# TIGER-AI-Lab/AnyV2V

Hardware: AMD Instinct MI355X
Metric: frames/sec for 16fx512x512 DDIM-inversion+PnP-edit; spatial-attn MFMA % of peak (higher is better)
Workload: dtype f16; 1 GPU; BASELINE config 3 per GPU: 1 clip x 16f x 512x512, 50-step DDIM inversion (UNet B=1) + 50-step PnP edit (UNet B=3, cfg 9.0, conv+spatial+temporal injection on every step); a bench step = 1 inversion step + 1 edit step = 1/50 clip; I2VGen-XL 3D-UNet 1.42B params, random init; frames=16, hip_graphs=True, finite=True

## Files before the change

### anyv2v_amd/csrc/gemm_plan.cpp

```cpp
#include "gemm_plan.h"

const char* av_gemm_family_name(GemmFamily f) {
    static const char* const names[] = {"naive", "ws", "ws_ln", "mfma128", "big", "pp", "sw", "sw_streamk", "swh"};
    static_assert(sizeof(names) / sizeof(names[0]) == GEMM_FAMILY_COUNT, "one name per family");
    return names[f];
}

namespace {
bool aligned16(const void* p) { return (((uintptr_t)p) & 15) == 0; }
int ceil_div(int a, int b) { return (a + b - 1) / b; }

#define PLAN_FAIL(code, ...) do { anyv2v_set_error(__VA_ARGS__); p.status = code; return p; } while (0)
#define PLAN_CHECK(cond, ...) if (!(cond)) PLAN_FAIL(ANYV2V_EINVAL, __VA_ARGS__)

int ws_slab_cols(const AnyV2VGemmDesc& d) {
    if (d.C0 == 320) return 160;
    if (d.C0 == 512) return d.act == ACT_GEGLU ? 128 : (d.N == 512 ? 64 : 0);
    return 0;
}
bool ws_eligible(const AnyV2VGemmDesc& d) {
    const int ns = ws_slab_cols(d);
    if (d.ln_c1 != nullptr && (d.R != nullptr || (d.C0 == 512 && d.act != ACT_GEGLU))) return false;
    return d.mode == MODE_LINEAR && ns > 0 && d.C1 == 0 && d.N % ns == 0 && d.N / ns <= 32 &&
           (d.act == ACT_NONE || (d.act == ACT_GEGLU && d.R == nullptr)) && d.rowvec == nullptr && d.M > 0;
}

bool sw_eligible(const AnyV2VGemmDesc& d, int nk) {
    const bool geglu = d.act == ACT_GEGLU;
    return d.N % 320 == 0 && (geglu ? d.mode == MODE_LINEAR && d.R == nullptr && d.rowvec == nullptr : d.act == ACT_NONE) &&
           !(d.R != nullptr && d.rowvec != nullptr) && nk >= 2 && d.ldc % 8 == 0 && (d.R == nullptr || d.ldr % 8 == 0) &&
           (d.rowvec == nullptr || d.ldrv % 8 == 0);
}
size_t sw_sk_workspace(int blocks) { return (size_t)2 * blocks * AV_GEMM_BM * AV_GEMM_BN * sizeof(float); }
int sw_sk_blocks(int tiles, int nk, bool force) {
    const long long U = (long long)tiles * nk;
    if (U < 256 * 4 || U > (1ll << 22)) return force && U >= 8 ? (int)(U / 4 < 256 ? U / 4 : 256) : 0;
    if (force) return 256;
    const int rounds = (tiles + 255) / 256;
    const double eff = (double)tiles / (rounds * 256.0);
    return eff < 0.9 ? 256 : 0;
}

bool swh_eligible(const AnyV2VGemmDesc& d) {
    return d.mode == MODE_CONV2D && d.stride == 1 && d.up == 0 && d.asym == 0 && d.Hi == d.Ho && d.Wi == d.Wo &&
           (d.Wi == 16 || d.Wi == 32 || d.Wi == 64) && d.N % 320 == 0 && d.act == ACT_NONE && d.C0 % 64 == 0 && d.C1 % 64 == 0 &&
           !(d.R != nullptr && d.rowvec != nullptr) && d.ldc % 8 == 0 && (d.R == nullptr || d.ldr % 8 == 0) &&
           (d.rowvec == nullptr || d.ldrv % 8 == 0);
}

bool gn_shape_ok(const AnyV2VGemmDesc& d) {
    if (d.gn_groups <= 0 || d.gn_rows_per_group <= 0 || d.N % 160 != 0 || d.N % d.gn_groups != 0) return false;
    const int cg = d.N / d.gn_groups;
    return 40 % cg == 0 && d.M % 16 == 0 && d.gn_rows_per_group % 16 == 0 && d.M % d.gn_rows_per_group == 0 &&
           (d.act == ACT_NONE || d.act == ACT_SILU || d.act == ACT_GELU);
}

void persistent_grid(GemmPlan& p, const AnyV2VGemmDesc& d) {
    p.tilesN = d.N / AV_GEMM_BN;
    p.tiles = ceil_div(d.M, AV_GEMM_BM) * p.tilesN;
    p.grid = p.tiles < 256 ? p.tiles : 256;
}
void raster(GemmPlan& p, const AnyV2VGemmDesc& d) {
    const int code = (d.flags >> ANYV2V_GEMM_RASTER_SHIFT) & 7;
    static const int gm_of[8] = {0, 0, 4, 8, 16, 32, 2, 0};
    int gm = gm_of[code];
    if (code == 0 && p.tilesN >= 8 && p.tiles >= 512) gm = 8;
    if (gm > 0 && p.grid == 256 && p.tilesN % (32 / gm) == 0) {
        p.rast_gm = gm;
        p.rast_gn = 32 / gm;
        p.rast_sm = ceil_div(ceil_div(d.M, AV_GEMM_BM), gm);
        p.rast_sn = p.tilesN / p.rast_gn;
        p.rast_nfast = (d.flags & ANYV2V_GEMM_RASTER_NFAST) != 0;
    }
}

}

GemmPlan av_gemm_plan(const AnyV2VGemmDesc& d, int hinted_rows) {
    GemmPlan p = {};
    p.nf = 4;
    p.splits = p.tilesN = 1;
    auto take = [&p](GemmFamily family, const char* what) { p.family = family; p.gn_decline = what; return p; };
    PLAN_CHECK(d.A0 && d.W, "gemm: null A0/W/C");
    PLAN_CHECK(d.M > 0 && d.N > 0 && d.C0 > 0 && d.C1 >= 0, "gemm: bad M/N/C0/C1 (%d %d %d %d)", d.M, d.N, d.C0, d.C1);
    PLAN_CHECK(d.mode >= 0 && d.mode <= 2, "gemm: bad mode %d", d.mode);
    PLAN_CHECK(d.act >= 0 && d.act <= 4, "gemm: bad act %d", d.act);
    PLAN_CHECK(d.act != ACT_F32OUT || (d.rowvec == nullptr && d.R == nullptr && d.N % 4 == 0 && d.ldc % 4 == 0),
               "gemm: fp32 output supports bias only and needs N, ldc multiples of 4");
    PLAN_CHECK(d.asym == 0 || d.asym == 1, "gemm: asym must be 0 or 1");
    PLAN_CHECK(d.C1 == 0 || d.A1 != nullptr, "gemm: C1 > 0 but A1 is null");
    PLAN_CHECK(d.rowvec == nullptr || d.rowvec_div > 0, "gemm: rowvec needs rowvec_div > 0");
    if (d.mode == MODE_CONV2D) {
        PLAN_CHECK(d.Hi > 0 && d.Wi > 0 && d.Ho > 0 && d.Wo > 0 && (d.stride == 1 || d.stride == 2), "gemm: bad conv geometry");
        PLAN_CHECK(d.M % (d.Ho * d.Wo) == 0, "gemm: M not a multiple of Ho*Wo");
        PLAN_CHECK(d.up == 0 || d.up == 1, "gemm: up must be 0 or 1");
    }
    if (d.mode == MODE_TEMPORAL) { PLAN_CHECK(d.F > 0 && d.HW > 0 && d.M % (d.F * d.HW) == 0, "gemm: bad temporal geometry"); }
    const bool geglu = d.act == ACT_GEGLU;
    if (geglu) {
        PLAN_CHECK(d.N % 32 == 0, "gemm: GEGLU needs N %% 32 == 0");
        PLAN_CHECK(d.rowvec == nullptr, "gemm: GEGLU with rowvec unsupported");
    }
    p.taps = d.mode == MODE_LINEAR ? 1 : (d.mode == MODE_CONV2D ? 9 : 3);
    p.nk = p.taps * (d.C0 / 64 + d.C1 / 64);
    p.vec_epi = (((uintptr_t)d.bias & 7) == 0) && (((uintptr_t)d.rowvec & 7) == 0) && (d.ldrv % 4 == 0) && (d.N % 4 == 0);
    const int flags = d.flags, nk = p.nk;
    const bool glds = (flags & ANYV2V_GEMM_LDS_DMA) != 0;
    const bool fast = !(flags & ANYV2V_GEMM_NAIVE) && d.C0 % 64 == 0 && d.C1 % 64 == 0 && d.lda0 % 8 == 0 &&
                      (d.C1 == 0 || d.lda1 % 8 == 0) && d.ldc % 8 == 0 && aligned16(d.A0) && (d.C1 == 0 || aligned16(d.A1)) &&
                      aligned16(d.W) && aligned16(d.C) && (d.R == nullptr || (d.ldr % 8 == 0 && aligned16(d.R))) &&
                      (!geglu || d.N % 128 == 0) && p.vec_epi;

    const bool ws_ok = fast && glds && ws_eligible(d);
    const bool ws_take = ws_ok && !(flags & (ANYV2V_GEMM_NO_WS | ANYV2V_GEMM_NO_BIG)) && (hinted_rows >= 32768 || (flags & ANYV2V_GEMM_FORCE_WS));
    if (d.ln_c1 != nullptr || ws_take) {
        p.grid = 256;
        if (ws_ok) p.tilesN = d.N / ws_slab_cols(d);
        if (d.ln_c1 == nullptr) return take(GEMM_WS, "the weight-stationary kernel");
        take(GEMM_WS_LN, "the LayerNorm-fold kernel");
        if (!(ws_ok && aligned16(d.ln_c1)))
            PLAN_FAIL(ANYV2V_EUNSUPPORTED, "gemm: ln_c1 (LayerNorm fold) needs mode 0, C0 = 320 (N %% 160 = 0) or C0 = 512 with GEGLU "
                      "(N %% 128 = 0), no residual / rowvec, 16-byte aligned operands -- got C0 %d N %d act %d", d.C0, d.N, d.act);
        return p;
    }
    if (!fast) {
        p.grid = (int)(unsigned)(((long long)d.M * (geglu ? d.N / 2 : d.N) + 255) / 256);
        return take(GEMM_NAIVE, "the naive kernel");
    }
    const bool sw_on = glds && !(flags & ANYV2V_GEMM_NO_SW);
    if (sw_on && (flags & (ANYV2V_GEMM_STREAMK | ANYV2V_GEMM_FORCE_STREAMK)) && sw_eligible(d, nk) && hinted_rows == d.M &&
        d.workspace != nullptr) {
        persistent_grid(p, d);
        const int blocks = sw_sk_blocks(p.tiles, nk, (flags & ANYV2V_GEMM_FORCE_STREAMK) != 0);
        if (blocks > 0 && sw_sk_workspace(blocks) <= (size_t)d.workspace_bytes) {
            p.grid = p.sk_blocks = blocks;
            return take(GEMM_SW_STREAMK, "the stream-K kernel");
        }
    }
    if (sw_on && (flags & ANYV2V_GEMM_SWH) && swh_eligible(d)) {
        persistent_grid(p, d);
        return take(GEMM_SWH, "the LDS-patch convolution kernel");
    }
    if (sw_on && (flags & ANYV2V_GEMM_SW) && sw_eligible(d, nk)) {
        persistent_grid(p, d);
        raster(p, d);
        return take(GEMM_SW, "the one-wave-per-SIMD kernel");
    }
    auto choose_nf = [&](int rows) -> int {
        int nf_ = geglu ? 4 : (d.N % 160 == 0 ? 5 : 4);
        if (!geglu && nf_ == 5 && d.N % 128 == 0) {
            const int mt = (rows + 127) / 128;
            const int t5 = mt * (d.N / 160), t4 = mt * (d.N / 128);
            const bool would_split = t4 < 384 && ((t4 <= 128 && nk >= 32) || nk >= 72);
            const bool prefer4 = !would_split && ((t4 <= 256) || (t5 > 256 && (t5 + 511) / 512 == (t4 + 511) / 512));
            if (((flags & ANYV2V_GEMM_NF4) || prefer4) && !(flags & ANYV2V_GEMM_NF5)) nf_ = 4;
        }
        return nf_;
    };
    const bool big_ok = glds && !(flags & ANYV2V_GEMM_NO_BIG) && d.N % 320 == 0 && (!geglu || d.mode == MODE_LINEAR) &&
                        (geglu || d.act == ACT_NONE);
    const size_t split_ws_bytes = (size_t)d.workspace_bytes < ((size_t)64 << 20) ? (size_t)d.workspace_bytes : ((size_t)64 << 20);
    struct Choice { bool big; int splits; };
    auto choose = [&](int rows) -> Choice {
        const bool ws_buf = d.workspace != nullptr && d.N % 8 == 0;
        if (big_ok) {
            const int tb = ceil_div(rows, AV_GEMM_BM) * (d.N / 320);
            const int rounds = (tb + 255) / 256;
            const bool fills = tb >= 224 && tb * 4 >= rounds * 256 * 3;
            if (!fills && !geglu && !(flags & (ANYV2V_GEMM_NO_SPLITK | ANYV2V_GEMM_FORCE_BIG)) && ws_buf && tb <= 128 && nk >= 72) {
                int sp = 256 / tb;
                if (sp > 8) sp = 8;
                if (sp > nk / 12) sp = nk / 12;
                if (sp >= 2 && tb * sp >= 224 && (size_t)sp * rows * d.N * sizeof(float) <= split_ws_bytes) return {true, sp};
            }
            if (fills || (flags & ANYV2V_GEMM_FORCE_BIG)) return {true, 1};
        }
        const int tm = ((rows + 127) / 128) * ceil_div(d.N, choose_nf(rows) * 32);
        const bool split_pays = (tm <= 128 && nk >= 32) || nk >= 72;
        if (glds && !geglu && d.act != ACT_F32OUT && !(flags & ANYV2V_GEMM_NO_SPLITK) && ws_buf && tm < 384 && split_pays) {
            int sp = (512 + tm - 1) / tm;
            if (sp > 8) sp = 8;
            if (sp > nk / 8) sp = nk / 8;
            if (sp >= 2 && (size_t)sp * rows * d.N * sizeof(float) <= split_ws_bytes) return {false, sp};
        }
        return {false, 1};
    };
    Choice use = choose(d.M);
    if (hinted_rows != d.M) {
        const Choice ref = choose(hinted_rows);
        if (ref.splits > 1)
            use = ref;
        else if (use.splits > 1)
            use = Choice{false, 1};
    }
    p.splits = use.splits;
    if (big_ok && !geglu && use.splits == 1 && !(flags & ANYV2V_GEMM_NO_PP) && (flags & ANYV2V_GEMM_PP)) {
        auto tiles_of = [&](int mf) { return ceil_div(d.M, 64 * mf) * (d.N / 320); };
        auto eff = [&](int mf) { return (double)tiles_of(mf) / (((tiles_of(mf) + 255) / 256) * 256.0); };
        p.pp_mf = (flags & ANYV2V_GEMM_PP_192) ? 3 : ((flags & ANYV2V_GEMM_PP_256) ? 4 : (eff(4) + 0.02 >= eff(3) ? 4 : 3));
        p.tilesN = d.N / 320;
        p.tiles = tiles_of(p.pp_mf);
        p.grid = p.tiles < 256 ? p.tiles : 256;
        return take(GEMM_PP, "the ping-pong kernel");
    }
    if (use.splits > 1)
// ... 23 lines not shown
```

### anyv2v_amd/csrc/gemm_ws.hip

```cpp
#include "gemm_common.h"

namespace {
constexpr int WS_RW = 32;
#ifndef WS_PRIO
#define WS_PRIO 1
#endif
}

template <int WS_K, int WS_NS, bool GEGLU, bool RES, int WS_R, int WQ, bool RR_EARLY, bool TRACE = false, bool LN = false>
__global__ __launch_bounds__(512) void gemm_ws_kernel(const GemmK p, const WsPlan plan) {
    constexpr int WS_KS = WS_K / 32;
    constexpr int WS_NF = WS_NS / 16;
    constexpr int WS_W_BYTES = (WS_K / 64) * WS_NS * 128;
    constexpr int WS_BIAS_BYTES = WS_NS * 2 + (LN ? WS_NS * 4 : 0);
    static_assert(!(LN && RES), "the LayerNorm-folded form has no residual epilogue (QKV / to_q / GEGLU take none)");
    constexpr int OUT_W = GEGLU ? WS_NS / 2 : WS_NS;
    constexpr int SLAB_LD = OUT_W + 8;
    constexpr int SLAB_BYTES = 16 * SLAB_LD * 2;
    constexpr int CPRW = OUT_W / 8;
    constexpr int NIT = (16 * CPRW + 63) / 64;
    __shared__ __attribute__((aligned(16))) char smem[WS_W_BYTES + WS_BIAS_BYTES + 8 * SLAB_BYTES];

    const int tid = threadIdx.x, lane = tid & 63;
    const int w = __builtin_amdgcn_readfirstlane(tid >> 6);
    const int l15 = lane & 15, lq = lane >> 4;
    const int xcd = blockIdx.x & 7, idx = blockIdx.x >> 3;
    if (idx >= plan.px * plan.S) return;
    const int slab = idx % plan.S;
    const int range = xcd * plan.px + idx / plan.S;
    const int s_begin = range * plan.spr;
    const int s_end = s_begin + plan.spr < plan.nstrips ? s_begin + plan.spr : plan.nstrips;
    const int n_wave = slab * WS_NS;

    auto a_row = [&](int strip, int mf) {
        int row = strip * WS_RW + mf * 16 + (lane >> 2);
        row = row < p.M ? row : p.M - 1;
        return p.A0 + (size_t)row * p.lda0 + (lane & 3) * 8;
    };
    const int bperm_addr = ((lane & 15) * 4 + (lane >> 4)) * 4;
    auto to_frag = [&](const h8& raw) {
        typedef int i4 __attribute__((ext_vector_type(4)));
        const i4 r = __builtin_bit_cast(i4, raw);
        i4 o;
#pragma unroll
        for (int i = 0; i < 4; ++i) o[i] = __builtin_amdgcn_ds_bpermute(bperm_addr, r[i]);
        return __builtin_bit_cast(h8, o);
    };
    h8 a[WS_R][2];
    int strip = s_begin + w;
    const half_t *pc0, *pc1;
    {
        const int s0 = strip < s_end ? strip : (s_begin < plan.nstrips ? s_begin : 0);
        pc0 = a_row(s0, 0);
        pc1 = a_row(s0, 1);
#pragma unroll
        for (int s = 0; s < WS_R; ++s) {
            a[s][0] = *(const h8*)(pc0 + s * 32);
            a[s][1] = *(const h8*)(pc1 + s * 32);
        }
    }
    {
        const half_t* wslab = p.W + (size_t)n_wave * WS_K;
        for (int j = w; j < (WS_K / 64) * (WS_NS / 8); j += 8) {
            const int kt = j / (WS_NS / 8), rg = j - kt * (WS_NS / 8);
            const int row = rg * 8 + (lane >> 3), kc = (lane & 7) ^ (row & 7);
            glds16(wslab + (size_t)row * WS_K + kt * 64 + kc * 8, smem + kt * (WS_NS * 128) + rg * 1024);
        }
        if (tid < WS_NS / 4) {
            const h4 b = *(const h4*)(p.bias != nullptr ? p.bias + n_wave + tid * 4 : p.zeros);
            *(h4*)(smem + WS_W_BYTES + tid * 8) = b;
            if constexpr (LN) *(f4*)(smem + WS_W_BYTES + WS_NS * 2 + tid * 16) = *(const f4*)(p.ln_c1 + n_wave + tid * 4);
        }
    }
    __syncthreads();

    const char* const wl = smem + l15 * 128;
    const int wsw[2] = {((0 * 4 + lq) ^ (l15 & 7)) * 16, ((1 * 4 + lq) ^ (l15 & 7)) * 16};
    half_t* const slabp = (half_t*)(smem + WS_W_BYTES + WS_BIAS_BYTES + w * SLAB_BYTES);
    const half_t* const bias_l = (const half_t*)(smem + WS_W_BYTES);
    const int n_out_wave = GEGLU ? n_wave / 2 : n_wave;
    static_assert(WS_KS % WS_R == 0 && WS_K % 64 == 0 && WS_NS % 16 == 0 && (!GEGLU || WS_NS % 32 == 0), "static ring indices need WS_R | WS_KS");
    static_assert(WS_W_BYTES + WS_BIAS_BYTES + 8 * SLAB_BYTES <= 160 * 1024, "W slab + epilogue slabs must fit in LDS");

    int nth = 0;
    if constexpr (TRACE) if (w >= plan.trace_waves) return;
    while (strip < s_end) {
        long long* tr = nullptr;
        if constexpr (TRACE) {
            if (nth == 2 && (w == 0 || w == (plan.trace_waves > 4 ? 4 : 1)) && lane == 0) tr = p.trace + ((size_t)blockIdx.x * 2 + (w != 0)) * 16;
            ++nth;
            if (tr) tr[0] = (long long)__builtin_amdgcn_s_memtime();
        }
        const int next = strip + 8;
        const int pre = next < s_end ? next : strip;
        const half_t* const pn0 = a_row(pre, 0);
        const half_t* const pn1 = a_row(pre, 1);
        const int m_wave = strip * WS_RW;
        h8 rr[2][RES ? NIT : 1];
        auto res_request = [&]() {
#pragma unroll
            for (int mf = 0; mf < 2; ++mf)
#pragma unroll
                for (int it = 0; it < (RES ? NIT : 0); ++it) {
                    const int c = it * 64 + lane;
                    const int row = c / CPRW, cc = c - row * CPRW;
                    int m = m_wave + mf * 16 + row;
                    m = m < p.M ? m : p.M - 1;
                    rr[mf][it] = *(const h8*)(p.R + (size_t)m * p.ldr + n_out_wave + cc * 8);
                }
        };
        if constexpr (RES && RR_EARLY) res_request();
        f4 acc[2][WS_NF];
#pragma unroll
        for (int i = 0; i < 2; ++i)
#pragma unroll
            for (int j = 0; j < WS_NF; ++j) {
                const h4 b = *(const h4*)(bias_l + j * 16 + 4 * lq);
                acc[i][j] = LN ? (f4){0.f, 0.f, 0.f, 0.f} : (f4){(float)b[0], (float)b[1], (float)b[2], (float)b[3]};
            }
        f4 accq[2] = {(f4){0.f, 0.f, 0.f, 0.f}, (f4){0.f, 0.f, 0.f, 0.f}}, accs[2] = {(f4){0.f, 0.f, 0.f, 0.f}, (f4){0.f, 0.f, 0.f, 0.f}};
        h8 ones;
#pragma unroll
        for (int e = 0; e < 8; ++e) ones[e] = (half_t)1.0f;

        constexpr int NFR = WS_KS * WS_NF;
        auto wfrag = [&](int idx) {
            const int s = idx / WS_NF, nf = idx - s * WS_NF;
            return *(const h8*)(wl + (s >> 1) * (WS_NS * 128) + wsw[s & 1] + nf * 2048);
        };
        auto request = [&](int t, int n) {
#pragma unroll
            for (int mf = 0; mf < 2; ++mf)
#pragma unroll
                for (int i = 0; i < n; ++i) {
                    const int u = t + i;
                    const half_t* q = u < WS_KS ? (mf ? pc1 : pc0) : (mf ? pn1 : pn0);
                    a[u % WS_R][mf] = *(const h8*)(q + (u < WS_KS ? u : u - WS_KS) * 32);
                }
        };
        constexpr bool PAIRS = WS_R % 2 == 0;
        h8 wq[WQ], fr[2][2];
#pragma unroll
        for (int i = 0; i < WQ - 1; ++i) wq[i] = wfrag(i);
        fr[0][0] = to_frag(a[0][0]);
        fr[0][1] = to_frag(a[0][1]);
        if (!PAIRS) request(WS_R, 1);
        if (WS_PRIO) __builtin_amdgcn_s_setprio(WS_PRIO);
        __builtin_amdgcn_sched_barrier(0);
#pragma unroll
        for (int s = 0; s < WS_KS; ++s)
#pragma unroll
        for (int nf = 0; nf < WS_NF; ++nf) {
            const int idx = s * WS_NF + nf;
            if (idx + WQ - 1 < NFR) wq[(idx + WQ - 1) % WQ] = wfrag(idx + WQ - 1);
            acc[0][nf] = __builtin_amdgcn_mfma_f32_16x16x32_f16(wq[idx % WQ], fr[s & 1][0], acc[0][nf], 0, 0, 0);
            acc[1][nf] = __builtin_amdgcn_mfma_f32_16x16x32_f16(wq[idx % WQ], fr[s & 1][1], acc[1][nf], 0, 0, 0);
            if constexpr (LN) {
                if (nf == 4 || nf == 5) {
                    accq[nf - 4] = __builtin_amdgcn_mfma_f32_16x16x32_f16(fr[s & 1][nf - 4], fr[s & 1][nf - 4], accq[nf - 4], 0, 0, 0);
                    accs[nf - 4] = __builtin_amdgcn_mfma_f32_16x16x32_f16(ones, fr[s & 1][nf - 4], accs[nf - 4], 0, 0, 0);
                }
            }
            if (nf == 2 && s + 1 < WS_KS) {
                fr[(s + 1) & 1][0] = to_frag(a[(s + 1) % WS_R][0]);
                fr[(s + 1) & 1][1] = to_frag(a[(s + 1) % WS_R][1]);
                if (!PAIRS) request(s + 1 + WS_R, 1);
                if (PAIRS && ((s + 1) & 1)) request(s + WS_R, 2);
            }
            if constexpr (TRACE) if (tr && nf == WS_NF - 1) tr[1 + s] = (long long)__builtin_amdgcn_s_memtime();
            __builtin_amdgcn_sched_barrier(0);
        }
        if (WS_PRIO) __builtin_amdgcn_s_setprio(0);
        pc0 = pn0;
        pc1 = pn1;
        if constexpr (RES && !RR_EARLY) res_request();

        int lane_e = lane;
        asm volatile("" : "+v"(lane_e));
        const int l15_e = lane_e & 15, lq_e = lane_e >> 4;
        float ln_mean[2] = {0.f, 0.f}, ln_rstd[2] = {1.f, 1.f};
        if constexpr (LN) {
#pragma unroll
            for (int mf = 0; mf < 2; ++mf) {
                const int r3 = l15_e & 3;
                float d = r3 == 0 ? accq[mf][0] : (r3 == 1 ? accq[mf][1] : (r3 == 2 ? accq[mf][2] : accq[mf][3]));
                d = __builtin_bit_cast(float, __builtin_amdgcn_ds_bpermute(((l15_e >> 2) * 16 + l15_e) * 4, __builtin_bit_cast(int, d)));
                const float mean = accs[mf][0] * (1.0f / WS_K);
                const float var = fmaxf(d * (1.0f / WS_K) - mean * mean, 0.0f);
                ln_mean[mf] = mean;
                ln_rstd[mf] = __builtin_amdgcn_rsqf(var + p.ln_eps);
            }
#pragma unroll
            for (int mf = 0; mf < 2; ++mf)
#pragma unroll
                for (int nf = 0; nf < WS_NF; ++nf) {
                    const f4 c1 = *(const f4*)((const char*)bias_l + WS_NS * 2 + (nf * 16 + 4 * lq_e) * 4);
                    const h4 b = *(const h4*)(bias_l + nf * 16 + 4 * lq_e);
#pragma unroll
                    for (int r = 0; r < 4; ++r)
                        acc[mf][nf][r] = fmaf(fmaf(-ln_mean[mf], c1[r], acc[mf][nf][r]), ln_rstd[mf], (float)b[r]);
                }
        }
#pragma unroll
        for (int mf = 0; mf < 2; ++mf) {
            if constexpr (GEGLU) {
#pragma unroll
                for (int np = 0; np < WS_NF / 2; ++np) {
                    h4 o;
#pragma unroll
                    for (int r = 0; r < 4; ++r)
                        o[r] = (half_t)(acc[mf][2 * np][r] * av_gelu(acc[mf][2 * np + 1][r]));
                    *(h4*)(slabp + l15_e * SLAB_LD + np * 16 + 4 * lq_e) = o;
                }
            } else {
#pragma unroll
                for (int nf = 0; nf < WS_NF; ++nf) {
                    h4 o;
#pragma unroll
                    for (int r = 0; r < 4; ++r) o[r] = (half_t)acc[mf][nf][r];
                    *(h4*)(slabp + l15_e * SLAB_LD + nf * 16 + 4 * lq_e) = o;
                }
            }
            if (RES && mf == 0) {
#pragma unroll
                for (int g = 0; g < 2; ++g)
#pragma unroll
                    for (int it = 0; it < NIT; ++it) asm volatile("" : "+v"(rr[g][RES ? it : 0]));
            }
#pragma unroll
            for (int it = 0; it < NIT; ++it) {
                const int c = it * 64 + lane_e;
                const int row = c / CPRW, cc = c - row * CPRW;
                const bool ok = (16 * CPRW % 64 == 0 || c < 16 * CPRW) && m_wave + mf * 16 + row < p.M;
                h8 v = *(const h8*)(slabp + (ok ? row * SLAB_LD + cc * 8 : 0));
                if constexpr (RES) v = v + rr[mf][it];
                if (ok) *(h8*)(p.C + (size_t)(m_wave + mf * 16 + row) * p.ldc + n_out_wave + cc * 8) = v;
            }
        }
        if constexpr (TRACE) if (tr) tr[11] = (long long)__builtin_amdgcn_s_memtime();
        __builtin_amdgcn_sched_barrier(0);
        strip = next;
    }
}

int av_gemm_ws_launch(const GemmK& k_in, const AnyV2VGemmDesc* d, const GemmPlan& gp, hipStream_t s) {
    GemmK k = k_in;
    WsPlan plan;
    plan.S = gp.tilesN;
    plan.px = 32 / plan.S;
    plan.nstrips = (d->M + WS_RW - 1) / WS_RW;
    const int nranges = 8 * plan.px;
    plan.spr = (plan.nstrips + nranges - 1) / nranges;
    plan.trace_waves = (d->flags & (1 << ANYV2V_GEMM_RASTER_SHIFT)) ? 4 : ((d->flags & (2 << ANYV2V_GEMM_RASTER_SHIFT)) ? 1 : 8);
    const bool geglu = d->act == ACT_GEGLU, res = d->R != nullptr;
#define WS_GO(K, NS, G, RS, R, Q, E, T) hipLaunchKernelGGL((gemm_ws_kernel<K, NS, G, RS, R, Q, E, T>), dim3(gp.grid), dim3(512), 0, s, k, plan)
#ifdef ANYV2V_EXPERIMENTS
    if ((d->flags & ANYV2V_GEMM_PROBE_TRACE) && d->C0 == 320 && d->workspace != nullptr && (size_t)256 * 2 * 16 * sizeof(long long) <= (size_t)d->workspace_bytes) {
        k.trace = (long long*)d->workspace;
        if (geglu) WS_GO(320, 160, true, false, 5, 8, false, true);
        else if (res) WS_GO(320, 160, false, true, 10, 4, false, true);
        else WS_GO(320, 160, false, false, 10, 4, false, true);
        return av_launch_status("gemm_ws<trace>");
    }
#endif
    if (gp.family == GEMM_WS_LN) {
#define WS_GO_LN(K, NS, G, R, Q) hipLaunchKernelGGL((gemm_ws_kernel<K, NS, G, false, R, Q, false, false, true>), dim3(gp.grid), dim3(512), 0, s, k, plan)
        if (d->C0 == 320) {
            if (geglu) WS_GO_LN(320, 160, true, 5, 4);
            else WS_GO_LN(320, 160, false, 10, 4);
        } else {
            WS_GO_LN(512, 128, true, 8, 4);
        }
#undef WS_GO_LN
        return av_launch_status("gemm_ws<LN>");
    }
    if (d->C0 == 320) {
        if (geglu) WS_GO(320, 160, true, false, 5, 8, false, false);
        else if (res) WS_GO(320, 160, false, true, 10, 4, false, false);
        else WS_GO(320, 160, false, false, 10, 4, false, false);
    } else {
        if (geglu) WS_GO(512, 128, true, false, 8, 8, false, false);
        else if (res) WS_GO(512, 64, false, true, 8, 4, false, false);
        else WS_GO(512, 64, false, false, 8, 8, false, false);
    }
#undef WS_GO
    return av_launch_status("gemm_ws");
}
```

### anyv2v_amd/ops.py

```python
from __future__ import annotations

import ctypes as C
import os
from typing import Optional

import torch

from . import _lib
from ._lib import AttnDesc, GemmDesc

MODE_LINEAR, MODE_CONV2D, MODE_TEMPORAL = 0, 1, 2
ACT_NONE, ACT_SILU, ACT_GELU, ACT_GEGLU, ACT_F32OUT = 0, 1, 2, 3, 4

FORCE_NAIVE = False
ATTN_FLAGS = int(os.environ.get("ANYV2V_ATTN_FLAGS", "0"))
GEMM_FLAGS = int(os.environ.get("ANYV2V_GEMM_FLAGS", "0"))
USE_GLDS = os.environ.get("ANYV2V_GLDS", "1") == "1"


def _parse_switch(value: Optional[str]) -> bool:
    return (value or "0").strip() == "1"


GN_EPILOGUE = _parse_switch(os.environ.get("ANYV2V_GN_EPILOGUE"))
# ... 97 lines not shown
    ws = _workspace(a0.device)
    d.workspace, d.workspace_bytes = ws.data_ptr(), ws.numel() * 4
    if gn is not None:
        stats, rows_per_group, groups = gn
        d.gn_rows_per_group, d.gn_groups = int(rows_per_group), int(groups)
        if stats is not None:
            assert stats.dtype == torch.float32 and stats.is_cuda and stats.is_contiguous()
            d.gn_stats, d.gn_stats_floats = stats.data_ptr(), stats.numel()
    if _query:
        return int(lib.anyv2v_gemm_gn_stats_floats(C.byref(d)))
    _lib.check(lib.anyv2v_gemm_f16(C.byref(d), _stream()), "anyv2v_gemm_f16")
    return out


def gemm_gn_stats_floats(a0: torch.Tensor, w: torch.Tensor, *, rows_per_group: int, groups: int = 32, **kw) -> int:
    return gemm(a0, w, gn=(None, rows_per_group, groups), _query=True, **kw)


def gn_launches(reset: bool = True) -> int:
    return int(_lib.load().anyv2v_gemm_gn_launches(int(reset)))


def gn_stats_floats(M: int, rows_per_group: int, groups: int = 32) -> int:
    return int(_lib.load().anyv2v_groupnorm_stats_floats(int(M), int(rows_per_group), int(groups)))


def groupnorm_from_stats(x: torch.Tensor, gamma, beta, stats: torch.Tensor, rows_per_group: int, *, groups: int = 32,
                         eps: float = 1e-5, silu: bool = False, out=None):
    lib = _lib.load()
    _rowmajor(x, "X")
    assert x.is_contiguous()
    M, Cc = x.shape
    if out is None:
        out = torch.empty((M, Cc), dtype=torch.float16, device=x.device)
    assert out.is_contiguous()
    assert stats.dtype == torch.float32 and stats.is_contiguous() and stats.numel() >= gn_stats_floats(M, rows_per_group, groups) > 0
    sizes = (C.c_int32 * 5)(M, Cc, rows_per_group, groups, min(stats.numel(), 2 ** 31 - 1))
    _lib.check(lib.anyv2v_groupnorm_apply_stats_f16(_p(x), _p(out), _p(gamma), _p(beta), _p(stats), sizes, eps, int(silu),
                                                    _stream()), "anyv2v_groupnorm_apply_stats_f16")
    return out


FF_FUSED = os.environ.get("ANYV2V_FF_FUSED", "1") == "1"


def ff_fused_supported(M: int, C: int, H: int) -> bool:
    return FF_FUSED and not FORCE_NAIVE and USE_GLDS and C == 320 and H == 1280 and M * _HINT[0] // _HINT[1] >= 32768


def ff_pack_w2(w2: torch.Tensor) -> torch.Tensor:
    C, H = w2.shape
    assert H % 32 == 0
    q, e = torch.arange(4).view(4, 1), torch.arange(8).view(1, 8)
    perm = torch.where(e < 4, 4 * q + e, 16 + 4 * q + (e - 4)).reshape(32).to(w2.device)
    return w2.view(C, H // 32, 32)[:, :, perm].permute(1, 0, 2).contiguous()


def ff_geglu(x: torch.Tensor, w1p: torch.Tensor, b1p: torch.Tensor, w2s: torch.Tensor, b2: torch.Tensor, residual=None, out=None):
    lib = _lib.load()
    M, Cc = x.shape
    H = w2s.shape[0] * 32
    assert x.dtype == torch.float16 and x.stride(1) == 1 and w1p.is_contiguous() and w2s.is_contiguous()
    assert tuple(w1p.shape) == (2 * H, Cc) and tuple(w2s.shape) == (H // 32, Cc, 32) and b1p.numel() == 2 * H and b2.numel() == Cc
    if out is None:
        out = torch.empty((M, Cc), dtype=torch.float16, device=x.device)
    for name, t in (("residual", residual), ("out", out)):
        assert t is None or (tuple(t.shape) == (M, Cc) and t.dtype == torch.float16 and t.stride(1) == 1 and t.device == x.device), \
            f"ff_geglu: {name} must be an fp16 [{M}, {Cc}] matrix with unit column stride on {x.device}"
    d = _lib.FFDesc()
    d.X, d.W1, d.b1, d.W2, d.b2, d.Y = _p(x), _p(w1p), _p(b1p), _p(w2s), _p(b2), _p(out)
    d.R = _p(residual) if residual is not None else None
    d.M, d.C, d.H = M, Cc, H
    d.ldx, d.ldy, d.ldr = x.stride(0), out.stride(0), (residual.stride(0) if residual is not None else 0)
    d.flags = d.reserved0 = 0
    _lib.check(lib.anyv2v_ff_geglu_f16(C.byref(d), _stream()), "anyv2v_ff_geglu_f16")
    return out


def ln_gemm_supported(M: int, K: int, N: int, act: int = ACT_NONE, hinted: bool = True) -> bool:
    if FORCE_NAIVE or not USE_GLDS or (GEMM_FLAGS & (_lib.ANYV2V_GEMM_NO_WS | _lib.ANYV2V_GEMM_NO_BIG)) or (M * _HINT[0] // _HINT[1] if hinted else M) < 32768:
        return False
    if K == 320:
        return N % 160 == 0 and N // 160 <= 32
    return K == 512 and act == ACT_GEGLU and N % 128 == 0 and N // 128 <= 32


def ln_fold(w: torch.Tensor, bias: Optional[torch.Tensor], gamma: torch.Tensor, beta: torch.Tensor):
    wf = w.float() * gamma.float()[None, :]
    w16 = wf.to(torch.float16).contiguous()
    c1 = w16.float().sum(1).contiguous()
    b = w.float() @ beta.float()
    if bias is not None:
        b = b + bias.float()
    return w16, b.to(torch.float16).contiguous(), c1


def gn_scratch_floats(M: int, rows_per_group: int, groups: int = 32) -> int:
    return (M // rows_per_group) * groups * 2 * 257


def groupnorm(x0: torch.Tensor, gamma, beta, stats: torch.Tensor, rows_per_group: int, *, x1=None, groups: int = 32,
              eps: float = 1e-5, silu: bool = False, out=None, shard=None):
    if shard is not None:
        return _groupnorm_sharded(x0, gamma, beta, stats, rows_per_group, x1, groups, eps, silu, out, shard)
    lib = _lib.load()
    _rowmajor(x0, "X0")
    assert x0.is_contiguous()
    M, C0 = x0.shape
    C1 = 0
    if x1 is not None:
        _rowmajor(x1, "X1")
        assert x1.is_contiguous() and x1.shape[0] == M
        C1 = x1.shape[1]
    if out is None:
        out = torch.empty((M, C0 + C1), dtype=torch.float16, device=x0.device)
    assert out.is_contiguous()
    need = gn_scratch_floats(M, rows_per_group, groups)
    assert stats.dtype == torch.float32 and stats.numel() >= need, "GroupNorm scratch too small"
    _lib.check(lib.anyv2v_groupnorm_f16(_p(x0), _p(x1), C0, C1, _p(out), _p(gamma), _p(beta), _p(stats), M,
                                        rows_per_group, groups, eps, int(silu), _stream()), "anyv2v_groupnorm_f16")
    return out


def _groupnorm_sharded(x0, gamma, beta, stats, rows_per_group, x1, groups, eps, silu, out, shard):
    lib = _lib.load()
    shards, all_reduce_sum = shard
    _rowmajor(x0, "X0")
    assert x0.is_contiguous()
    M, C0 = x0.shape
    C1 = 0
    if x1 is not None:
        _rowmajor(x1, "X1")
        assert x1.is_contiguous() and x1.shape[0] == M
        C1 = x1.shape[1]
    if out is None:
        out = torch.empty((M, C0 + C1), dtype=torch.float16, device=x0.device)
    assert out.is_contiguous()
    n = int(lib.anyv2v_groupnorm_partial_floats(M, rows_per_group, groups, C0 + C1))
    npiv = (M // rows_per_group) * groups
    assert n > 0 and stats.dtype == torch.float32 and stats.numel() >= n + npiv, "GroupNorm scratch too small"
    piv = stats[n:n + npiv]
    _lib.check(lib.anyv2v_groupnorm_pivot_f16(_p(x0), _p(x1), C0, C1, _p(piv), M, rows_per_group, groups, int(shards), _stream()),
               "anyv2v_groupnorm_pivot_f16")
    all_reduce_sum(piv)
    _lib.check(lib.anyv2v_groupnorm_partial_pivot_f16(_p(x0), _p(x1), C0, C1, _p(piv), _p(stats), M, rows_per_group, groups,
                                                      _stream()), "anyv2v_groupnorm_partial_pivot_f16")
    all_reduce_sum(stats[:n])
    _lib.check(lib.anyv2v_groupnorm_apply_pivot_f16(_p(x0), _p(x1), C0, C1, _p(out), _p(gamma), _p(beta), _p(piv), _p(stats), M,
                                                    rows_per_group, groups, eps, int(silu), int(shards), _stream()),
               "anyv2v_groupnorm_apply_pivot_f16")
    return out


def layernorm(x: torch.Tensor, gamma, beta, eps: float = 1e-5, out=None):
    lib = _lib.load()
    _rowmajor(x, "X")
    assert x.is_contiguous()
    M, Cc = x.shape
    if out is None:
        out = torch.empty_like(x)
    _lib.check(lib.anyv2v_layernorm_f16(_p(x), _p(out), _p(gamma), _p(beta), M, Cc, eps, _stream()), "anyv2v_layernorm_f16")
    return out


def softmax_rows(s: torch.Tensor, scale: float, out: Optional[torch.Tensor] = None):
    lib = _lib.load()
    assert s.dim() == 2 and s.stride(1) == 1 and s.dtype == torch.float32 and s.is_cuda
# ... 466 lines not shown
```

### anyv2v_amd/unet.py

```python
from __future__ import annotations

import copy
import math
import os

from dataclasses import dataclass
from typing import List, Optional, Tuple

import torch
import torch.nn as nn

from . import ops
from .ops import ACT_GEGLU, ACT_GELU, ACT_NONE, ACT_SILU, MODE_CONV2D, MODE_TEMPORAL


@dataclass
class I2VGenXLUNetConfig:
    in_channels: int = 4
    out_channels: int = 4
    block_out_channels: Tuple[int, ...] = (320, 640, 1280, 1280)
    layers_per_block: int = 2
    norm_num_groups: int = 32
    cross_attention_dim: int = 1024
    attention_head_dim: int = 64
# ... 282 lines not shown
        return self._run_foreign(proc, ctx, h, geom, residual, kv)

    def _run_foreign(self, proc, ctx, h, geom: Geom, residual, kv):
        C = h.shape[1]
        if geom.kind == "spatial":
            hs = h.view(geom.batch, geom.S, C)
        else:
            hs = h.view(geom.B, geom.F, geom.HW, C).permute(0, 2, 1, 3).reshape(geom.batch, geom.S, C)
        ehs = None
        if kv is not None:
            ehs = ctx.context.view(ctx.B, ctx.Sk, -1).repeat_interleave(geom.F, dim=0)
        out = proc(self, hs, encoder_hidden_states=ehs)
        if geom.kind != "spatial":
            out = out.view(geom.B, geom.HW, geom.F, C).permute(0, 2, 1, 3)
        out = out.reshape(-1, C).contiguous()
        return ops.add(out, residual)


class GEGLU(nn.Module):
    def __init__(self, dim_in, dim_out):
        super().__init__()
        self.proj = Linear(dim_in, dim_out * 2)
        self.dim_out = dim_out
        self._w = self._b = None

    def pack(self):
        w, b = self.proj.weight.data, self.proj.bias.data
        n = self.dim_out
        assert n % 16 == 0
        wh, wg = w[:n].view(n // 16, 16, -1), w[n:].view(n // 16, 16, -1)
        self._w = torch.stack([wh, wg], 1).reshape(2 * n, -1).contiguous()
        bh, bg = b[:n].view(n // 16, 16), b[n:].view(n // 16, 16)
        self._b = torch.stack([bh, bg], 1).reshape(2 * n).contiguous()


class GELUProj(nn.Module):
    def __init__(self, dim_in, dim_out):
        super().__init__()
        self.proj = Linear(dim_in, dim_out)


class FeedForward(nn.Module):
    def __init__(self, dim, inner_dim=None, activation_fn="geglu"):
        super().__init__()
        inner_dim = inner_dim or dim * 4
        self.geglu = activation_fn == "geglu"
        act = GEGLU(dim, inner_dim) if self.geglu else GELUProj(dim, inner_dim)
        self.net = nn.ModuleList([act, Identity(), Linear(inner_dim, dim)])

    def pack(self):
        lin = self.net[2]
        self._w2s = ops.ff_pack_w2(lin.weight.data) if (self.geglu and tuple(lin.weight.shape) == (320, 1280)) else None

    def run(self, h, residual, ln_in=None):
        w2s = getattr(self, "_w2s", None)
        if ln_in is None and w2s is not None and ops.ff_fused_supported(h.shape[0], h.shape[1], w2s.shape[0] * 32):
            return ops.ff_geglu(h, self.net[0]._w, self.net[0]._b, w2s, self.net[2].bias, residual=residual)
        if ln_in is not None:
            x, (w_in, b_in, c1_in), ln_eps = ln_in
            g = ops.gemm(x, w_in, bias=b_in, act=ACT_GEGLU, ln=(c1_in, ln_eps))
        elif self.geglu:
            g = ops.gemm(h, self.net[0]._w, bias=self.net[0]._b, act=ACT_GEGLU)
        else:
            g = ops.gemm(h, self.net[0].proj.weight, bias=self.net[0].proj.bias, act=ACT_GELU)
        return ops.gemm(g, self.net[2].weight, bias=self.net[2].bias, residual=residual)


class BasicTransformerBlock(nn.Module):
    def __init__(self, dim, heads, dim_head, cross_attention_dim=None, double_self_attention=False):
        super().__init__()
        self.norm1 = LayerNorm(dim)
        self.attn1 = Attention(dim, None, heads, dim_head)
        self.norm2 = LayerNorm(dim)
        self.attn2 = Attention(dim, None if double_self_attention else cross_attention_dim, heads, dim_head)
        self.norm3 = LayerNorm(dim)
        self.ff = FeedForward(dim)

    def pack(self):
        self._ln = {}
        dim = self.norm1.weight.shape[0]
        if dim not in (320, 512) or _NO_LN_FOLD:
            return
        cat = lambda a: torch.cat([a.to_q.weight.data, a.to_k.weight.data, a.to_v.weight.data], 0)
        if dim == 320:
            self._ln["attn1"] = ops.ln_fold(cat(self.attn1), None, self.norm1.weight.data, self.norm1.bias.data)
            w2 = self.attn2.to_q.weight.data if self.attn2.is_cross else cat(self.attn2)
            self._ln["attn2"] = ops.ln_fold(w2, None, self.norm2.weight.data, self.norm2.bias.data)
        if self.ff.geglu and _LN_FOLD_FF:
            g = self.ff.net[0]
            w, b, c1 = ops.ln_fold(g.proj.weight.data, g.proj.bias.data, self.norm3.weight.data, self.norm3.bias.data)
            n = g.dim_out
            il = lambda t: torch.stack([t[:n].reshape(n // 16, 16, *t.shape[1:]), t[n:].reshape(n // 16, 16, *t.shape[1:])], 1) \
                .reshape(2 * n, *t.shape[1:]).contiguous()
            self._ln["ff"] = (il(w), il(b), il(c1))

    def _fold(self, name, proc_ok, M, N, act=ACT_NONE, per_branch=False):
        f = getattr(self, "_ln", {}).get(name)
        return f if (f is not None and proc_ok and ops.ln_gemm_supported(M, self.norm1.weight.shape[0], N, act, hinted=not per_branch)) else None

    def run(self, ctx, x, geom: Geom, expand=None, shrink=None):
        dim = x.shape[1]
        rows_b = lambda t, g: t.shape[0] // g.B
        f = self._fold("attn1", isinstance(self.attn1.processor, HipAttnProcessor), rows_b(x, geom), 3 * dim, per_branch=True)
        if f is not None:
            x = self.attn1.run(ctx, None, geom, residual=x, ln_in=(x, f, self.norm1.eps))
        else:
            h = ops.layernorm(x, self.norm1.weight, self.norm1.bias, self.norm1.eps)
            x = self.attn1.run(ctx, h, geom, residual=x)
        if expand is not None:
            after = getattr(ctx, "batch_hint_after", None)
            ctx, geom = expand
            x = expand_shared(x, ctx)
            if after is not None:
                ops.set_batch_hint(*after)
        if shrink is not None:
            x = x[x.shape[0] // 3:]
            geom = shrink
            ops.set_batch_hint(3, 2)
        kv = ctx.kv_for(self.attn2) if self.attn2.is_cross else None
        f = self._fold("attn2", isinstance(self.attn2.processor, HipAttnProcessor), rows_b(x, geom), dim if self.attn2.is_cross else 3 * dim,
                       per_branch=True)
        if f is not None:
            x = self.attn2.run(ctx, None, geom, residual=x, kv=kv, ln_in=(x, f, self.norm2.eps))
        else:
            h = ops.layernorm(x, self.norm2.weight, self.norm2.bias, self.norm2.eps)
            x = self.attn2.run(ctx, h, geom, residual=x, kv=kv)
        f = self._fold("ff", True, x.shape[0], 8 * dim, ACT_GEGLU)
        if f is not None:
            return self.ff.run(None, residual=x, ln_in=(x, f, self.norm3.eps))
        h = ops.layernorm(x, self.norm3.weight, self.norm3.bias, self.norm3.eps)
        return self.ff.run(h, residual=x)


class Transformer2DModel(nn.Module):
    def __init__(self, heads, dim_head, in_channels, cross_attention_dim, groups):
        super().__init__()
        inner = heads * dim_head
        self.norm = GroupNorm(groups, in_channels, eps=1e-6)
        self.proj_in = Linear(in_channels, inner)
        self.transformer_blocks = nn.ModuleList([BasicTransformerBlock(inner, heads, dim_head, cross_attention_dim)])
        self.proj_out = Linear(inner, in_channels)

    def run(self, ctx, x, H, W, full_ctx=None):
        HW = H * W
        h = ops.groupnorm(x, self.norm.weight, self.norm.bias, ctx.stats, HW, groups=self.norm.num_groups,
                          eps=self.norm.eps)
        h = ops.gemm(h, self.proj_in.weight, bias=self.proj_in.bias)
        geom = Geom("spatial", ctx.B, ctx.F, HW)
        for i, blk in enumerate(self.transformer_blocks):
            if full_ctx is not None and i == 0:
                h = blk.run(ctx, h, geom, expand=(full_ctx, Geom("spatial", full_ctx.B, full_ctx.F, HW)))
                ctx, geom = full_ctx, Geom("spatial", full_ctx.B, full_ctx.F, HW)
                x = expand_shared(x, full_ctx)
            else:
                h = blk.run(ctx, h, geom)
        return ops.gemm(h, self.proj_out.weight, bias=self.proj_out.bias, residual=x)


class TransformerTemporalModel(nn.Module):
    def __init__(self, heads, dim_head, in_channels, groups):
        super().__init__()
        inner = heads * dim_head
        self.norm = GroupNorm(groups, in_channels, eps=1e-6)
        self.proj_in = Linear(in_channels, inner)
        self.transformer_blocks = nn.ModuleList(
            [BasicTransformerBlock(inner, heads, dim_head, None, double_self_attention=True)])
        self.proj_out = Linear(inner, in_channels)

    def run(self, ctx, x, H, W):
        fp = getattr(ctx, "fp", None)
        return self._run(ctx, x, H * W, None) if fp is None else fp.temporal(ctx, x, H * W, self._run)

    def _run(self, ctx, x, HW, shard):
        h = ops.groupnorm(x, self.norm.weight, self.norm.bias, ctx.stats, ctx.F * HW, groups=self.norm.num_groups,
                          eps=self.norm.eps, shard=shard)
        h = ops.gemm(h, self.proj_in.weight, bias=self.proj_in.bias)
        geom = Geom("temporal", ctx.B, ctx.F, HW)
        drop = shard is None and getattr(ctx, "drop_tail_at", None) is self and not self.transformer_blocks[0].attn2.is_cross
        for i, blk in enumerate(self.transformer_blocks):
            if drop and i == 0:
# ... 565 lines not shown
```

Measured before the change: 3.037 frames/s.

## Extend LayerNorm-fold WS GEMM to 512-dim QKV and widen residual slab

Extends the weight-stationary LayerNorm-folded GEMM to C0=512 with N=1536 (fused QKV for the 512-channel transformer blocks) using 96-column slabs, and enables the LN fold for dim 512 attn1/attn2 unless PnP injection is active on that step. It also switches the residual C0=512, N=512 path to 128-column slabs with a two-turn epilogue that writes the output in halves to keep LDS staging small. The aim is to remove separate LayerNorm passes and to halve the number of slab passes over A for the residual projection. The cost is more accumulator registers per wave and extra epilogue complexity. Since PnP injection runs on every step, the fold is bypassed for the edit pass and the change only helps the inversion pass and any non-injected blocks.

```diff
diff --git a/anyv2v_amd/csrc/gemm_plan.cpp b/anyv2v_amd/csrc/gemm_plan.cpp
--- a/anyv2v_amd/csrc/gemm_plan.cpp
+++ b/anyv2v_amd/csrc/gemm_plan.cpp
@@ -15,12 +15,16 @@
 
 int ws_slab_cols(const AnyV2VGemmDesc& d) {
     if (d.C0 == 320) return 160;
-    if (d.C0 == 512) return d.act == ACT_GEGLU ? 128 : (d.N == 512 ? 64 : 0);
+    if (d.C0 == 512) {
+        if (d.act == ACT_GEGLU) return 128;
+        if (d.N == 512) return d.R != nullptr ? 128 : 64;
+        if (d.N == 1536 && d.ln_c1 != nullptr && d.R == nullptr) return 96;
+    }
     return 0;
 }
 bool ws_eligible(const AnyV2VGemmDesc& d) {
     const int ns = ws_slab_cols(d);
-    if (d.ln_c1 != nullptr && (d.R != nullptr || (d.C0 == 512 && d.act != ACT_GEGLU))) return false;
+    if (d.ln_c1 != nullptr && (d.R != nullptr || (d.C0 == 512 && d.act != ACT_GEGLU && d.N != 1536))) return false;
     return d.mode == MODE_LINEAR && ns > 0 && d.C1 == 0 && d.N % ns == 0 && d.N / ns <= 32 &&
            (d.act == ACT_NONE || (d.act == ACT_GEGLU && d.R == nullptr)) && d.rowvec == nullptr && d.M > 0;
 }
@@ -119,8 +123,9 @@
         if (d.ln_c1 == nullptr) return take(GEMM_WS, "the weight-stationary kernel");
         take(GEMM_WS_LN, "the LayerNorm-fold kernel");
         if (!(ws_ok && aligned16(d.ln_c1)))
-            PLAN_FAIL(ANYV2V_EUNSUPPORTED, "gemm: ln_c1 (LayerNorm fold) needs mode 0, C0 = 320 (N %% 160 = 0) or C0 = 512 with GEGLU "
-                      "(N %% 128 = 0), no residual / rowvec, 16-byte aligned operands -- got C0 %d N %d act %d", d.C0, d.N, d.act);
+            PLAN_FAIL(ANYV2V_EUNSUPPORTED, "gemm: ln_c1 (LayerNorm fold) needs mode 0, C0 = 320 (N %% 160 = 0) or C0 = 512 (GEGLU with "
+                      "N %% 128 = 0, or N = 1536), no residual / rowvec, 16-byte aligned operands -- got C0 %d N %d act %d",
+                      d.C0, d.N, d.act);
         return p;
     }
     if (!fast) {
diff --git a/anyv2v_amd/csrc/gemm_ws.hip b/anyv2v_amd/csrc/gemm_ws.hip
--- a/anyv2v_amd/csrc/gemm_ws.hip
+++ b/anyv2v_amd/csrc/gemm_ws.hip
@@ -7,7 +7,7 @@
 #endif
 }
 
-template <int WS_K, int WS_NS, bool GEGLU, bool RES, int WS_R, int WQ, bool RR_EARLY, bool TRACE = false, bool LN = false>
+template <int WS_K, int WS_NS, bool GEGLU, bool RES, int WS_R, int WQ, bool RR_EARLY, bool TRACE = false, bool LN = false, int TURNS = 1>
 __global__ __launch_bounds__(512) void gemm_ws_kernel(const GemmK p, const WsPlan plan) {
     constexpr int WS_KS = WS_K / 32;
     constexpr int WS_NF = WS_NS / 16;
@@ -15,10 +15,12 @@
     constexpr int WS_BIAS_BYTES = WS_NS * 2 + (LN ? WS_NS * 4 : 0);
     static_assert(!(LN && RES), "the LayerNorm-folded form has no residual epilogue (QKV / to_q / GEGLU take none)");
     constexpr int OUT_W = GEGLU ? WS_NS / 2 : WS_NS;
-    constexpr int SLAB_LD = OUT_W + 8;
+    constexpr int TURN_W = OUT_W / TURNS;
+    constexpr int SLAB_LD = TURN_W + 8;
     constexpr int SLAB_BYTES = 16 * SLAB_LD * 2;
-    constexpr int CPRW = OUT_W / 8;
+    constexpr int CPRW = TURN_W / 8;
     constexpr int NIT = (16 * CPRW + 63) / 64;
+    static_assert(OUT_W % (16 * TURNS) == 0 && (!LN || WS_NF >= 6), "whole fragments per turn; the LayerNorm statistics ride on fragments 4 and 5");
     __shared__ __attribute__((aligned(16))) char smem[WS_W_BYTES + WS_BIAS_BYTES + 8 * SLAB_BYTES];
 
     const int tid = threadIdx.x, lane = tid & 63;
@@ -96,17 +98,17 @@
         const half_t* const pn0 = a_row(pre, 0);
         const half_t* const pn1 = a_row(pre, 1);
         const int m_wave = strip * WS_RW;
-        h8 rr[2][RES ? NIT : 1];
+        h8 rr[2][RES ? TURNS * NIT : 1];
         auto res_request = [&]() {
 #pragma unroll
             for (int mf = 0; mf < 2; ++mf)
 #pragma unroll
-                for (int it = 0; it < (RES ? NIT : 0); ++it) {
-                    const int c = it * 64 + lane;
+                for (int ti = 0; ti < (RES ? TURNS * NIT : 0); ++ti) {
+                    const int tn = ti / NIT, c = (ti - tn * NIT) * 64 + lane;
                     const int row = c / CPRW, cc = c - row * CPRW;
                     int m = m_wave + mf * 16 + row;
                     m = m < p.M ? m : p.M - 1;
-                    rr[mf][it] = *(const h8*)(p.R + (size_t)m * p.ldr + n_out_wave + cc * 8);
+                    rr[mf][ti] = *(const h8*)(p.R + (size_t)m * p.ldr + n_out_wave + tn * TURN_W + cc * 8);
                 }
         };
         if constexpr (RES && RR_EARLY) res_request();
@@ -202,30 +204,33 @@
                 }
         }
 #pragma unroll
-        for (int mf = 0; mf < 2; ++mf) {
+        for (int mf = 0; mf < 2; ++mf)
+#pragma unroll
+        for (int tn = 0; tn < TURNS; ++tn) {
+            constexpr int NFT = (GEGLU ? WS_NF / 2 : WS_NF) / TURNS;
             if constexpr (GEGLU) {
 #pragma unroll
-                for (int np = 0; np < WS_NF / 2; ++np) {
+                for (int np = tn * NFT; np < (tn + 1) * NFT; ++np) {
                     h4 o;
 #pragma unroll
                     for (int r = 0; r < 4; ++r)
                         o[r] = (half_t)(acc[mf][2 * np][r] * av_gelu(acc[mf][2 * np + 1][r]));
-                    *(h4*)(slabp + l15_e * SLAB_LD + np * 16 + 4 * lq_e) = o;
+                    *(h4*)(slabp + l15_e * SLAB_LD + (np - tn * NFT) * 16 + 4 * lq_e) = o;
                 }
             } else {
 #pragma unroll
-                for (int nf = 0; nf < WS_NF; ++nf) {
+                for (int nf = tn * NFT; nf < (tn + 1) * NFT; ++nf) {
                     h4 o;
 #pragma unroll
                     for (int r = 0; r < 4; ++r) o[r] = (half_t)acc[mf][nf][r];
-                    *(h4*)(slabp + l15_e * SLAB_LD + nf * 16 + 4 * lq_e) = o;
-                }
-            }
-            if (RES && mf == 0) {
+                    *(h4*)(slabp + l15_e * SLAB_LD + (nf - tn * NFT) * 16 + 4 * lq_e) = o;
+                }
+            }
+            if (RES && mf == 0 && tn == 0) {
 #pragma unroll
                 for (int g = 0; g < 2; ++g)
 #pragma unroll
-                    for (int it = 0; it < NIT; ++it) asm volatile("" : "+v"(rr[g][RES ? it : 0]));
+                    for (int ti = 0; ti < TURNS * NIT; ++ti) asm volatile("" : "+v"(rr[g][RES ? ti : 0]));
             }
 #pragma unroll
             for (int it = 0; it < NIT; ++it) {
@@ -233,8 +238,8 @@
                 const int row = c / CPRW, cc = c - row * CPRW;
                 const bool ok = (16 * CPRW % 64 == 0 || c < 16 * CPRW) && m_wave + mf * 16 + row < p.M;
                 h8 v = *(const h8*)(slabp + (ok ? row * SLAB_LD + cc * 8 : 0));
-                if constexpr (RES) v = v + rr[mf][it];
-                if (ok) *(h8*)(p.C + (size_t)(m_wave + mf * 16 + row) * p.ldc + n_out_wave + cc * 8) = v;
+                if constexpr (RES) v = v + rr[mf][RES ? tn * NIT + it : 0];
+                if (ok) *(h8*)(p.C + (size_t)(m_wave + mf * 16 + row) * p.ldc + n_out_wave + tn * TURN_W + cc * 8) = v;
             }
         }
         if constexpr (TRACE) if (tr) tr[11] = (long long)__builtin_amdgcn_s_memtime();
@@ -268,8 +273,10 @@
         if (d->C0 == 320) {
             if (geglu) WS_GO_LN(320, 160, true, 5, 4);
             else WS_GO_LN(320, 160, false, 10, 4);
+        } else if (geglu) {
+            WS_GO_LN(512, 128, true, 8, 4);
         } else {
-            WS_GO_LN(512, 128, true, 8, 4);
+            WS_GO_LN(512, 96, false, 8, 4);
         }
 #undef WS_GO_LN
         return av_launch_status("gemm_ws<LN>");
@@ -280,7 +287,7 @@
         else WS_GO(320, 160, false, false, 10, 4, false, false);
     } else {
         if (geglu) WS_GO(512, 128, true, false, 8, 8, false, false);
-        else if (res) WS_GO(512, 64, false, true, 8, 4, false, false);
+        else if (res) hipLaunchKernelGGL((gemm_ws_kernel<512, 128, false, true, 8, 4, false, false, false, 2>), dim3(gp.grid), dim3(512), 0, s, k, plan);
         else WS_GO(512, 64, false, false, 8, 8, false, false);
     }
 #undef WS_GO
diff --git a/anyv2v_amd/ops.py b/anyv2v_amd/ops.py
--- a/anyv2v_amd/ops.py
+++ b/anyv2v_amd/ops.py
@@ -203,7 +203,9 @@
         return False
     if K == 320:
         return N % 160 == 0 and N // 160 <= 32
-    return K == 512 and act == ACT_GEGLU and N % 128 == 0 and N // 128 <= 32
+    if K == 512 and act == ACT_GEGLU:
+        return N % 128 == 0 and N // 128 <= 32
+    return K == 512 and N == 1536
 
 
 def ln_fold(w: torch.Tensor, bias: Optional[torch.Tensor], gamma: torch.Tensor, beta: torch.Tensor):
diff --git a/anyv2v_amd/unet.py b/anyv2v_amd/unet.py
--- a/anyv2v_amd/unet.py
+++ b/anyv2v_amd/unet.py
@@ -388,10 +388,9 @@
         if dim not in (320, 512) or _NO_LN_FOLD:
             return
         cat = lambda a: torch.cat([a.to_q.weight.data, a.to_k.weight.data, a.to_v.weight.data], 0)
-        if dim == 320:
-            self._ln["attn1"] = ops.ln_fold(cat(self.attn1), None, self.norm1.weight.data, self.norm1.bias.data)
-            w2 = self.attn2.to_q.weight.data if self.attn2.is_cross else cat(self.attn2)
-            self._ln["attn2"] = ops.ln_fold(w2, None, self.norm2.weight.data, self.norm2.bias.data)
+        self._ln["attn1"] = ops.ln_fold(cat(self.attn1), None, self.norm1.weight.data, self.norm1.bias.data)
+        w2 = self.attn2.to_q.weight.data if self.attn2.is_cross else cat(self.attn2)
+        self._ln["attn2"] = ops.ln_fold(w2, None, self.norm2.weight.data, self.norm2.bias.data)
         if self.ff.geglu and _LN_FOLD_FF:
             g = self.ff.net[0]
             w, b, c1 = ops.ln_fold(g.proj.weight.data, g.proj.bias.data, self.norm3.weight.data, self.norm3.bias.data)
@@ -402,6 +401,11 @@
 
     def _fold(self, name, proc_ok, M, N, act=ACT_NONE, per_branch=False):
         f = getattr(self, "_ln", {}).get(name)
+        dim = self.norm1.weight.shape[0]
+        if f is not None and proc_ok and dim == 512 and name != "ff":
+            p = getattr(self, name).processor
+            if pnp_on(p.t, p.injection_schedule):
+                return None
         return f if (f is not None and proc_ok and ops.ln_gemm_supported(M, self.norm1.weight.shape[0], N, act, hinted=not per_branch)) else None
 
     def run(self, ctx, x, geom: Geom, expand=None, shrink=None):
```

After: 3.050 frames/s (median of 6 runs). Within noise of the previous version (+0.4%).
